# cure-lab/MotionCraft

Measured on AMD Instinct MI355X. Metric: sampled SMPL-X frames/sec (196-frame seq, 1000-step DDPM), higher is better.
Workload: dtype f32

## Files before the change

motioncraft_amd/csrc/mc_ctx.h:

```cpp
#pragma once
#include <map>
#include <mutex>
#include <string>
#include <vector>

#include "../../include/motioncraft_amd.h"
#include "mc_common.h"
#include "mc_gemm.h"
#include "mc_kernels.h"
#include "mc_chain.h"
#include "mc_half.h"
#include "mc_options.h"
#include "mc_params.h"

struct mc_model {
    mc_model_config cfg;
    ParamStore params{""};
    std::map<std::string, HalfW> half;
    std::mutex half_mu;
    size_t half_bytes = 0;
    bool finalized = false;
    int Cp = 0;
};

// ... 40 lines not shown
    const float* mask = nullptr;
    float* mask_own = nullptr;
    int* t_orig;
    float *te, *e1, *emb, *semb, *ss;
    RouteBufs rb;
    int device = 0;
    int coop_reserved = 0;
    bool prof_on = false;
    std::vector<ProfRec> prof;
    bool have_cond = false;
    hipStream_t side = nullptr;
    bool xpad_ready = false;
    hipEvent_t ev_fork = nullptr, ev_join = nullptr;
    hipEvent_t ev_side = nullptr;
    hipEvent_t ev_stag = nullptr;
    bool no_alias = false;
    bool defer_last_gemm = false;
    static constexpr int SIDE_CAND = 4;
    hipStream_t side_cand[SIDE_CAND] = {nullptr, nullptr, nullptr, nullptr};
    hipStream_t side_for = nullptr;
    bool side_picked = false;
    float side_probe_ms[SIDE_CAND] = {0.f, 0.f, 0.f, 0.f};
    static constexpr int SIDE_MEMO = 4;
    hipStream_t side_memo_for[SIDE_MEMO] = {nullptr, nullptr, nullptr, nullptr};
    int side_memo_pick[SIDE_MEMO] = {-1, -1, -1, -1};
    int side_memo_n = 0;
    int* gstep = nullptr;
    SamplerCoefs* gcoefs = nullptr;
    bool graph_mode = false;
    hipGraph_t graph = nullptr;
// ... 37 lines not shown
```

motioncraft_amd/csrc/mc_kernels.h:

```cpp
#pragma once
#include <hip/hip_runtime.h>
#include <stdint.h>
#include "mc_options.h"

struct TwinAlias {
    const int* split_flag = nullptr;
    long from = 0;
};

int mc_launch_ln_rows(const float* X, long ldx, int x_col, const float* gamma, const float* beta,
                      const float* add, int add_mod, float* Y, long ldy, long rows, int L, hipStream_t s);
struct StepRef {
    const int* ptr = nullptr;
    long stride = 0;
};
int mc_launch_film_rows(const float* Y1, const float* Y2, const float* gamma, const float* beta,
                        const float* ss, float* A, long rows, int D, hipStream_t s, TwinAlias y1_alias = TwinAlias(), long row0 = 0,
                        StepRef step = StepRef(), int y1_parts = 1, long y1_pstride = 0,
                        int planes = 0, long plane_stride = 0);
int mc_launch_timestep_embedding(const int* t_orig, float* te, int S, int D, hipStream_t s);
int mc_launch_silu(const float* X, float* Y, long n, hipStream_t s);
int mc_launch_add_rows(float* out, const float* a, const float* b, const float* bias, long rows, int D, hipStream_t s);
int mc_launch_softmax_rows_small(const float* W, float* out, int rows, int cols, hipStream_t s);

// ... 67 lines not shown
    int max_tiles;
    uint32_t tie_xor = 0xFFFFFFFFu;
};
size_t mc_route_state_ints(int E);
bool mc_route_is_small(const McOptions& o, long N);
bool mc_route_cleans_counts(const McOptions& o, long N);
size_t mc_route_barrier_offset();
size_t mc_route_error_offset();
int mc_route_coop_wgs(long N);
int mc_route_coop_slots(int dev);
bool mc_route_coop_reserve(int dev, int nwg);
void mc_route_coop_release(int dev, int nwg);
size_t mc_route_barrier_ints();
int mc_launch_gate_finish(const float* proj, const float* sim_n, const float* logit_scale, long N, int E,
                          RouteBufs rb, hipStream_t s);
int mc_launch_route(long N, long Nsrc, long gsplit, int E, int capacity, RouteBufs rb, const McOptions& o, hipStream_t s);
const int* mc_route_num_tiles_ptr(const RouteBufs& rb, int group = 0);
const int* mc_route_split_flag_ptr(const RouteBufs& rb);

int mc_launch_body(const float* mf, long ldmf, const float* qkv, const float* wsm, float* ys,
                   long frames, int H, int L, int G, hipStream_t s, TwinAlias alias = TwinAlias(), long frame0 = 0);
int mc_launch_temporal(const float* mf, const float* tf, const float* mask, float* yt,
                       int b0, int nb, int B, int T, int Nt, int H, int L, hipStream_t s, const int* twin_flag = nullptr,
                       long lsplit_max = 96,
                       bool pair = false,
                       bool skip_text = false);
```

motioncraft_amd/csrc/mc_model.hip:

```cpp
#include "mc_ctx.h"

namespace {

template <class T>
int ws_alloc(mc_ctx* c, T** p, size_t n) {
    void* d = nullptr;
    size_t bytes = (n * sizeof(T) + 255) & ~(size_t)255;
    if (bytes == 0) bytes = 256;
    MC_HIP(hipMalloc(&d, bytes));
    c->allocs.push_back(d);
    c->bytes += (int64_t)bytes;
    *p = (T*)d;
    return MC_OK;
}

int bind_moe(const mc_model* m, const std::string& pre, int din, int dout, int seq_rows, MoeW* w) {
    const int64_t E = m->cfg.num_experts;
    w->din = din;
    w->dout = dout;
    return m->params.bind({{&w->emb, pre + "emb", (int64_t)seq_rows * din},       {&w->gate_w, pre + "gate_w", 256 * din},
                           {&w->gate_b, pre + "gate_b", 256},                      {&w->sim_n, pre + "sim_n", 256 * E},
                           {&w->sim_nT, pre + "sim_nT", 32 * 256},                 {&w->scale, pre + "scale", 1},
                           {&w->fc1_w, pre + "fc1_w", E * 4 * din * din},          {&w->fc1_b, pre + "fc1_b", E * 4 * din},
                           {&w->fc2_wt, pre + "fc2_wt", E * din * 4 * din},        {&w->fc2_b, pre + "fc2_b", E * din},
// ... 162 lines not shown
    {"temporal_split", "MC_TEMPORAL_SPLIT", nullptr, &McOptions::temporal_split, 96},
    {"big_tokens", "MC_BIG_TOKENS", nullptr, &McOptions::big_tokens, 65536},
    {"rowchain_split", "MC_ROWCHAIN_SPLIT", nullptr, &McOptions::rowchain_split, 20480},
    {"gemm_tune", "MC_GEMM_TUNE", nullptr, &McOptions::gemm_tune, kTuneDefault, check_tune},
    {"small_tile_n", "MC_SMALL_TILE_N", nullptr, &McOptions::small_tile_n, 0,
     [](long v) -> std::string { return v == 0 || v == 48 || v == 64 || v == 96 ? "" : "small_tile_n: 0 (per-launch choice), 48, 64 or 96"; }},
    {"gemm_wp_grid", "MC_GEMM_WP_GRID", nullptr, &McOptions::gemm_wp_grid, 512},
    {"half_min_rows", "MC_HALF_MIN_ROWS", nullptr, &McOptions::half_min_rows, 512},
    {"gate_small", "MC_GATE_SMALL", nullptr, &McOptions::gate_small, 12000},
    {"split_expert", "MC_SPLIT_EXPERT", nullptr, &McOptions::split_expert, 0},
    {"split_sffn", "MC_SPLIT_SFFN", nullptr, &McOptions::split_sffn, 0},
    {"route_reg", "MC_ROUTE_REG", nullptr, &McOptions::route_reg, 1},
    {"route_coop", "MC_ROUTE_COOP", nullptr, &McOptions::route_coop, 1, nullptr, route_coop_hook},
    {"route_small", "MC_ROUTE_SMALL_CTX", "MC_ROUTE_SMALL", &McOptions::route_small, 20480,
     [](long v) -> std::string { return v >= 0 && v <= 131072 ? "" : "route_small: 0 .. 131072 pairs (the one-workgroup kernels hold at most 131072)"; }},
    {"route_per", nullptr, nullptr, &McOptions::route_per, 0,
     [](long v) -> std::string { return v == 0 || v == 10 || v == 16 ? "" : "route_per: 0 (default), 10 or 16"; }},
    {"dbg_delay_us", nullptr, nullptr, &McOptions::dbg_delay_us, 0,
     [](long v) -> std::string { return v >= -100000 && v <= 100000 ? "" : "dbg_delay_us: -100000 .. 100000"; }},
};

int seed_options(McOptions& o) {
    for (const OptionDef& d : kOptions) {
        const char *var = nullptr, *e = nullptr;
        for (const char* v : {d.env, d.env_alt})
            if (v && !e && (e = getenv(v))) var = v;
        const std::string why = e && d.check ? d.check(atol(e)) : "";
        MC_REQUIRE(why.empty(), "%s=%s: %s", var, e, why.c_str());
        o.*d.field = e ? atol(e) : d.dflt;
    }
// ... 59 lines not shown
    probe.m = m;
    int r = bind_weights(&probe);
    if (r != MC_OK) return r;
    m->finalized = true;
    return MC_OK;
}

int mc_ctx_create(mc_model* m, int32_t batch, int32_t frames, int32_t max_steps, mc_ctx** out) {
    MC_REQUIRE(m && out, "null argument");
    MC_REQUIRE(m->finalized, "model not finalized");
    MC_REQUIRE(batch >= 1 && frames >= 1 && frames <= m->cfg.max_seq_len, "bad batch/frames (%d, %d)", batch, frames);
    MC_REQUIRE(max_steps >= 1, "max_steps < 1");
    const mc_model_config& g = m->cfg;
    mc_ctx* c = new mc_ctx();
    if (int r = seed_options(c->opt)) { mc_ctx_destroy(c); return r; }
    c->m = m;
    c->B = batch;
    c->T = frames;
    c->maxS = max_steps;
    const int L = g.latent_dim, H = g.num_parts, D = L * H, F = g.ffn_dim, Te = g.time_embed_dim, Dt = g.text_latent_dim;
    const long B2 = 2L * batch;
    c->rows = B2 * frames;
    c->N = c->rows * H;
    c->Ntxt = B2 * g.max_text_len;
    int r = bind_weights(c);
    if (r == MC_OK) r = build_ctx_weights(c);
    if (r != MC_OK) { mc_ctx_destroy(c); return r; }
    bool cand_ok = true;
    for (int k = 0; k < mc_ctx::SIDE_CAND; ++k) cand_ok = cand_ok && hipStreamCreateWithFlags(&c->side_cand[k], hipStreamNonBlocking) == hipSuccess;
    c->side = c->side_cand[0];
    for (hipEvent_t* e : {&c->ev_fork, &c->ev_join, &c->ev_side, &c->ev_stag}) cand_ok = cand_ok && hipEventCreateWithFlags(e, hipEventDisableTiming) == hipSuccess;
    if (!cand_ok) {
        mc_set_error("could not create the side stream / events");
        mc_ctx_destroy(c);
        return MC_ERR_HIP;
    }
    const long Nmax = c->N > c->Ntxt ? c->N : c->Ntxt;
    const size_t zsz = (size_t)(c->N * L > c->Ntxt * Dt ? c->N * L : c->Ntxt * Dt);
    const size_t hsz = (size_t)(2 * c->N * 4 * L > 2 * c->Ntxt * 4 * Dt ? 2 * c->N * 4 * L : 2 * c->Ntxt * 4 * Dt);
#define WS(p, n) do { if ((r = ws_alloc(c, &(p), (size_t)(n))) != MC_OK) { mc_ctx_destroy(c); return r; } } while (0)
    WS(c->h, c->rows * D);
    WS(c->z, zsz);
    WS(c->proj, Nmax * 256);
    WS(c->hbuf, hsz);
    c->hbuf_cap = hsz;
    if (chain_on(c, kChainMlp) && mc_mlp_supported(L, 4 * L)) c->hbuf_floats = hsz;
// ... 51 lines not shown
    c->graph_multistep = false;
    c->graph_k1.clear();
}
static void prof_clear(mc_ctx* c) {
    for (auto& p : c->prof) { if (p.e0) (void)hipEventDestroy(p.e0); if (p.e1) (void)hipEventDestroy(p.e1); }
    c->prof.clear();
}

void mc_ctx_destroy(mc_ctx* c) {
    if (!c) return;
    graph_release(c);
    if (c->coop_reserved) { mc_route_coop_release(c->device, c->coop_reserved); c->coop_reserved = 0; }
    prof_clear(c);
    for (int k = 0; k < mc_ctx::SIDE_CAND; ++k)
        if (c->side_cand[k]) { (void)hipStreamSynchronize(c->side_cand[k]); (void)hipStreamDestroy(c->side_cand[k]); }
    for (hipEvent_t e : {c->ev_fork, c->ev_join, c->ev_side, c->ev_stag})
        if (e) (void)hipEventDestroy(e);
    for (void* p : c->allocs) (void)hipFree(p);
    delete c;
}

int64_t mc_ctx_workspace_bytes(const mc_ctx* c) { return c ? (int64_t)(c->bytes + (c->prec != MC_PREC_F32 ? c->m->half_bytes : 0)) : 0; }

int mc_ctx_check(mc_ctx* c, void* stream) {
    MC_REQUIRE(c, "null context");
    int flag = 0;
    MC_HIP(hipMemcpyAsync(&flag, c->rb.state + mc_route_error_offset(), sizeof(int), hipMemcpyDeviceToHost, (hipStream_t)stream));
    MC_HIP(hipStreamSynchronize((hipStream_t)stream));
    if (flag != 0) {
        mc_set_error("the cooperative routing kernel's grid barrier timed out (its workgroups were not all resident: another process "
                     "is holding the GPU with barrier kernels of its own); the results of this context are invalid -- destroy it and "
// ... 409 lines not shown
    else if (n == "emb") { p = c->emb; cnt = (int64_t)c->S * g.time_embed_dim; }
    else if (n == "ss") { p = c->ss + (long)layer * c->maxS * 2 * D; cnt = (int64_t)c->S * 2 * D; }
    else if (n == "tf") { p = c->tf + (long)layer * c->Ntxt * 2 * L; cnt = c->Ntxt * 2 * L; }
    else if (n == "idx") { p = c->rb.idx; cnt = 2 * c->N; }
    else if (n == "gate") { p = c->rb.gate; cnt = 2 * c->N; }
    else if (n == "comb_w") { p = c->rb.comb_w; cnt = 2 * c->N; }
    else if (n == "key") { p = c->rb.key; cnt = c->N; }
    else if (n == "hc" && c->hc) { p = c->hc; cnt = c->rows * D; }
    else if (n == "cb" && c->cb) { p = c->cb; cnt = c->rows * D; }
    else if (n == "cap_idx" && c->cap_idx) { p = c->cap_idx + (long)layer * 2 * c->N; cnt = 2 * c->N; }
    else if (n == "cap_w" && c->cap_w) { p = c->cap_w + (long)layer * 2 * c->N; cnt = 2 * c->N; }
    else if (n == "x0_hist") {
        if (!c->x0_hist) { mc_set_error("buffer 'x0_hist' does not exist before the context's first multistep (mode 2) call"); return MC_ERR_STATE; }
        p = c->x0_hist; cnt = (int64_t)c->B * c->T * g.input_feats;
    }
    else if (n == "route_split") { p = const_cast<int*>(mc_route_split_flag_ptr(c->rb)); cnt = 1; }
    else { mc_set_error("unknown buffer '%s'", name); return MC_ERR_ARG; }
    *dev_ptr = p;
    *numel = cnt;
    return MC_OK;
}

int mc_op_gemm(const float* a, const float* w, const float* bias, const float* res, float* cdev, int32_t M, int32_t N,
               int32_t K, int32_t ldw, int32_t act, void* stream) {
    MC_REQUIRE(a && w && cdev && M > 0 && N > 0 && K > 0 && K % 4 == 0 && ldw % 4 == 0 && ldw >= K, "bad gemm args");
    return dense(nullptr, a, K, w, ldw, bias, res, N, cdev, N, M, N, K, act, (hipStream_t)stream);
}

int mc_op_gemm_strided(int32_t mode, int32_t groups, const mc_gemm_strided* a, void* stream) {
    MC_REQUIRE(a && (mode == GM_PLAIN || mode == GM_ENC) && groups >= 1, "gemm_strided: mode %d (0 plain, 4 encoder), groups %d", mode, groups);
// ... 125 lines not shown
```

motioncraft_amd/csrc/mc_options.h:

```cpp
#pragma once

enum ChainBit {
    kChainMlp = 0,
    kChainGate = 1,
    kChainRowchain = 2,
    kChainTwin = 4,
    kChainTwoStreams = 5,
    kChainGroupExperts = 6,
    kChainDeferTail = 7,
    kChainTwinAlias = 8,
    kChainCtrlGroups = 9,
    kChainProjQkv = 10,
    kChainTailGrouped = 11,
    kChainSffnPartials = 12,
    kChainDynSlices = 13,
    kChainSideBody = 14,
    kChainPqBody = 15,
    kChainTwinSplit = 16,
    kChainFilmPlanes = 17,
    kChainMlpDma = 18,
    kChainPadX = 19,
    kChainTemporalHalf = 20,
    kChainTailOnePass = 21,
    kChainTemporalPair = 22,
    kChainSkipText = 24,
    kChainStagger = 26,
    kChainResidualPre = 27,
    kChainFragMajor = 29,
    kChainBits = 30,
};
constexpr long kChainRetired = 1L << 3 | 1L << 23 | 1L << 25 | 1L << 28;
constexpr long kChainDefault = ((1L << kChainBits) - 1) & ~kChainRetired;
static_assert(kChainDefault == 763363319, "the default chain mask is public ABI");

struct McOptions {
    long chain, small_gemm_rows, split_rows_expert, split_rows_sffn, temporal_split, big_tokens, rowchain_split;
    long gemm_tune, small_tile_n, gemm_wp_grid, half_min_rows, gate_small, split_expert, split_sffn;
    long route_reg, route_coop, route_small, route_per, dbg_delay_us;
};

const McOptions* mc_process_options();
```

motioncraft_amd/csrc/mc_route.hip:

```cpp
#include "mc_common.h"
#include "mc_kernels.h"
#include <stdlib.h>

namespace {

constexpr int MAXE = 16;
constexpr int MAXP = 2 * MAXE;
constexpr int TILE_ROWS = 128;

enum {
    ST_CNT = 0,
    ST_KEPT = ST_CNT + MAXP,
    ST_FILL = ST_KEPT + 2 * MAXE,
    ST_OFF = ST_FILL + 2 * MAXE,
    ST_ACTIVE = ST_OFF + 2 * MAXE + 1,
    ST_RANK = ST_ACTIVE + MAXP,
    ST_ANY = ST_RANK + MAXP,
    ST_NTILES = ST_ANY + 1,
    ST_DONE = ST_NTILES + 2,
    ST_SPLIT = ST_DONE + 1,
    ST_PREFIX = ST_DONE + 2,
    ST_HIST = ST_PREFIX + 2 * MAXP,
    ST_BAR = (ST_HIST + MAXP * 256 + 31) / 32 * 32,
    ST_TOTAL = ST_BAR + 17 * 32
};

__device__ __forceinline__ unsigned long long composite(uint32_t key, uint32_t tok, uint32_t tie_xor) {
    return ((unsigned long long)key << 32) | (unsigned long long)(tok ^ tie_xor);
}

__global__ __launch_bounds__(256) void gate_finish_k(const float* __restrict__ proj, const float* __restrict__ sim_n,
                                                     const float* __restrict__ logit_scale, long N, int E,
                                                     int* __restrict__ idx, float* __restrict__ gate,
                                                     uint32_t* __restrict__ key, int* __restrict__ state) {
    __shared__ float s_sim[256 * MAXE];
    __shared__ int s_cnt[MAXP];
    for (int i = threadIdx.x; i < 256 * MAXE; i += 256) {
        const int j = i / MAXE, e = i % MAXE;
// ... 28 lines not shown
        if (e == 0) {
            const float den = fmaxf(m1 + m2, 1.1920928955078125e-07f);
            idx[tok * 2] = c1;
            idx[tok * 2 + 1] = c2;
            gate[tok * 2] = m1 / den;
            gate[tok * 2 + 1] = m2 / den;
            key[tok] = __float_as_uint(m1);
            atomicAdd(&s_cnt[c1], 1);
            atomicAdd(&s_cnt[MAXE + c2], 1);
        }
    }
    __syncthreads();
    if (threadIdx.x < MAXP && s_cnt[threadIdx.x]) atomicAdd(&state[ST_CNT + threadIdx.x], s_cnt[threadIdx.x]);
}

__global__ void route_init_k(int* __restrict__ state, int E, int capacity, int cnt_mul) {
    const int p = threadIdx.x;
    __shared__ int any;
    if (p == 0) any = 0;
    __syncthreads();
    if (p < MAXP) {
        const int choice = p / MAXE, e = p % MAXE;
        int act = 0, rank = 0;
        if (e < E) {
            const int c0 = state[ST_CNT + e] * cnt_mul;
            const int cnt = state[ST_CNT + p] * cnt_mul;
            const int limit = choice == 0 ? capacity : capacity - c0;
            if (limit <= 0) act = cnt > 0 ? -1 : 0;
            else if (cnt > limit) { act = 1; rank = limit; }
        }
        state[ST_ACTIVE + p] = act;
        state[ST_RANK + p] = rank;
        state[ST_PREFIX + 2 * p] = 0;
        state[ST_PREFIX + 2 * p + 1] = 0;
        if (act == 1) atomicOr(&any, 1);
    }
    for (int i = threadIdx.x; i < MAXP * 256; i += blockDim.x) state[ST_HIST + i] = 0;
    if (threadIdx.x < 2 * MAXE) { state[ST_KEPT + threadIdx.x] = 0; state[ST_FILL + threadIdx.x] = 0; }
    if (threadIdx.x < 2) state[ST_DONE + threadIdx.x] = 0;
    __syncthreads();
    if (p == 0) state[ST_ANY] = any;
}

__global__ __launch_bounds__(256) void route_hist_k(const int* __restrict__ idx, const uint32_t* __restrict__ key,
                                                    long N, long Nsrc, int* __restrict__ state, int pass, uint32_t tie_xor) {
    if (state[ST_ANY] == 0) return;
    __shared__ int h[MAXP * 256];
    __shared__ int s_act[MAXP];
    __shared__ unsigned long long s_pre[MAXP];
    for (int i = threadIdx.x; i < MAXP * 256; i += 256) h[i] = 0;
    if (threadIdx.x < MAXP) {
        s_act[threadIdx.x] = state[ST_ACTIVE + threadIdx.x];
        s_pre[threadIdx.x] = ((unsigned long long)(uint32_t)state[ST_PREFIX + 2 * threadIdx.x] << 32) |
                             (uint32_t)state[ST_PREFIX + 2 * threadIdx.x + 1];
    }
    __syncthreads();
// ... 142 lines not shown
            lp[i] = atomicAdd(&s_cnt[le[i]], 1);
        }
    }
    __syncthreads();
    if (threadIdx.x < 2 * MAXE && s_cnt[threadIdx.x])
        s_base[threadIdx.x] = state[ST_OFF + threadIdx.x] + atomicAdd(&state[ST_FILL + threadIdx.x], s_cnt[threadIdx.x]);
    __syncthreads();
#pragma unroll
    for (int i = 0; i < PER; ++i) {
        if (le[i] >= 0) {
            const long a = a0 + i;
            const int slot = s_base[le[i]] + lp[i];
            src_row[slot] = (int)(a >> 1);
            dst_row[slot] = (int)a;
        }
    }
}

__device__ __forceinline__ int ld_state(const int* p) { return __hip_atomic_load(p, __ATOMIC_RELAXED, __HIP_MEMORY_SCOPE_AGENT); }

constexpr int BAR_STRIDE = 32, BAR_INTS = 17 * BAR_STRIDE;
constexpr unsigned BAR_SPIN_LIMIT = 1u << 23;
template <class F>
__device__ __forceinline__ bool grid_sync(int* bar, int nwg, int* s_last, int* s_gen, F&& last_hook) {
    const int grp = (int)(blockIdx.x & 7), ngrp = nwg < 8 ? nwg : 8, members = (nwg - grp + 7) >> 3;
    int* cnt = bar + BAR_STRIDE * (1 + grp);
    int* gen = bar + BAR_STRIDE * (9 + grp);
    __syncthreads();
    if (threadIdx.x == 0) {
        *s_gen = __hip_atomic_load(gen, __ATOMIC_RELAXED, __HIP_MEMORY_SCOPE_AGENT);
// ... 589 lines not shown
    cached[dev].store(v);
    return v;
}
bool mc_route_coop_reserve(int dev, int nwg) {
    if (nwg <= 0 || dev < 0 || dev >= 64) return false;
    const int slots = mc_route_coop_slots(dev);
    int cur = g_coop_reserved[dev].load();
    while (cur + nwg <= slots)
        if (g_coop_reserved[dev].compare_exchange_weak(cur, cur + nwg)) return true;
    return false;
}
void mc_route_coop_release(int dev, int nwg) {
    if (nwg > 0 && dev >= 0 && dev < 64) g_coop_reserved[dev].fetch_sub(nwg);
}
const int* mc_route_num_tiles_ptr(const RouteBufs& rb, int group) { return rb.state + ST_NTILES + group; }
const int* mc_route_split_flag_ptr(const RouteBufs& rb) { return rb.state + ST_SPLIT; }

int mc_launch_gate_finish(const float* proj, const float* sim_n, const float* logit_scale, long N, int E,
                          RouteBufs rb, hipStream_t s) {
    MC_REQUIRE(E >= 2 && E <= MAXE, "gate: num_experts=%d unsupported (2..16)", E);
    MC_HIP(hipMemsetAsync(rb.state, 0, sizeof(int) * (ST_CNT + MAXP), s));
    int blocks = cdiv(N, 16);
    if (blocks > 4096) blocks = 4096;
    hipLaunchKernelGGL(gate_finish_k, dim3(blocks), dim3(256), 0, s, proj, sim_n, logit_scale, N, E, rb.idx, rb.gate,
                       rb.key, rb.state);
    MC_LAUNCH_CHECK();
    return MC_OK;
}

int mc_launch_route(long N, long Nsrc, long gsplit, int E, int capacity, RouteBufs rb, const McOptions& o, hipStream_t s) {
    MC_REQUIRE(Nsrc == N || 2 * Nsrc == N, "route: Nsrc=%ld must be N or N/2 (N=%ld)", Nsrc, N);
    MC_REQUIRE(Nsrc == N || rb.tie_xor == 0xFFFFFFFFu, "route: the twin mode needs the stable tie order (a twin must rank right behind its original)");
    if (mc_route_is_small(o, N)) {
#define MC_ROUTE_SMALL(KERNEL)                                                                                                       \
    hipLaunchKernelGGL(KERNEL, dim3(1), dim3(SMALL_THREADS), 0, s, rb.idx, rb.gate, rb.key, N, Nsrc, gsplit, E, capacity,   \
                       (int)(N / Nsrc), rb.comb_w, rb.state, rb.src_row, rb.dst_row, rb.tile_group, rb.tile_row0, rb.tile_nrows,        \
                       rb.max_tiles, rb.tie_xor)
        if (o.route_reg && 2 * N <= 10L * SMALL_THREADS) MC_ROUTE_SMALL(route_small_k<10>);
        else if (o.route_reg && 2 * N <= 20L * SMALL_THREADS) MC_ROUTE_SMALL(route_small_k<20>);
        else MC_ROUTE_SMALL(route_small_stream_k);
#undef MC_ROUTE_SMALL
        MC_LAUNCH_CHECK();
        return MC_OK;
    }
    if (o.route_coop && 2 * N <= COOP_MAX_WG * 256 * COOP_PER) {
        const int per = o.route_per ? (int)o.route_per : (cdiv(2 * N, 256L * COOP_PER) > 256 ? 16 : 10);
        const int nwg = cdiv(2 * N, 256L * per);
#define MC_ROUTE_COOP(P)                                                                                                             \
    hipLaunchKernelGGL(route_coop_k<P>, dim3(nwg), dim3(256), 0, s, rb.idx, rb.gate, rb.key, N, Nsrc, gsplit, E, capacity, (int)(N / Nsrc), \
                       rb.comb_w, rb.state, rb.src_row, rb.dst_row, rb.tile_group, rb.tile_row0, rb.tile_nrows, rb.max_tiles, rb.tie_xor,  \
                       N <= 65536 ? 1 : 0)
        if (per == 16) MC_ROUTE_COOP(16); else MC_ROUTE_COOP(10);
#undef MC_ROUTE_COOP
        MC_LAUNCH_CHECK();
        return MC_OK;
    }
    hipLaunchKernelGGL(route_init_k, dim3(1), dim3(256), 0, s, rb.state, E, capacity, (int)(N / Nsrc));
    int blocks = cdiv(2 * N, 256 * 8);
    if (blocks > 1024) blocks = 1024;
    if (blocks < 1) blocks = 1;
    for (int pass = 0; pass < 8; ++pass) {
        hipLaunchKernelGGL(route_hist_k, dim3(blocks), dim3(256), 0, s, rb.idx, rb.key, N, Nsrc, rb.state, pass, rb.tie_xor);
    }
    hipLaunchKernelGGL(route_keep_k, dim3(blocks), dim3(256), 0, s, rb.idx, rb.gate, rb.key, N, Nsrc, gsplit, rb.comb_w, rb.state, rb.tie_xor);
    hipLaunchKernelGGL(route_plan_k, dim3(1), dim3(256), 0, s, rb.state, E, rb.tile_group, rb.tile_row0, rb.tile_nrows,
                       rb.max_tiles);
    hipLaunchKernelGGL(route_fill_k, dim3(cdiv(2 * Nsrc, 256 * 8)), dim3(256), 0, s, rb.idx, rb.comb_w, Nsrc, gsplit, rb.state,
                       rb.src_row, rb.dst_row);
    MC_LAUNCH_CHECK();
    return MC_OK;
}
```

motioncraft_amd/csrc/mc_step.hip:

```cpp
#include "mc_ctx.h"

bool use_half(const mc_ctx* c) { return c->prec != MC_PREC_F32 && c->rows > c->opt.half_min_rows; }
static const HalfW* half_planes(const mc_ctx* c, const HalfW* hw) { return hw && hw->hi && use_half(c) ? hw : nullptr; }
static bool split3(const mc_ctx* c) { return c->prec == MC_PREC_F16X3; }

static bool twin_aliased(const mc_ctx* c, bool twin) { return twin && chain_on(c, kChainTwinAlias) && !c->no_alias; }
static TwinAlias twin_alias(const mc_ctx* c, bool twin, bool tokens) {
    return twin_aliased(c, twin) ? TwinAlias{mc_route_split_flag_ptr(c->rb), (tokens ? c->N : c->rows) / 2} : TwinAlias();
}

template <class Args>
static void set_tile_map(const mc_ctx* c, int group, Args& a) {
    const long to = (long)group * c->rb.max_tiles;
    a.tile_group = c->rb.tile_group + to; a.tile_row0 = c->rb.tile_row0 + to; a.tile_nrows = c->rb.tile_nrows + to;
    a.num_tiles = mc_route_num_tiles_ptr(c->rb, group);
}

static int dbg_hold(const mc_ctx* c, hipStream_t pos, hipStream_t neg) {
    const long us = c->opt.dbg_delay_us;
    return us == 0 ? MC_OK : mc_launch_spin((us > 0 ? us : -us) * 100, us > 0 ? pos : neg);
}

int dense(const mc_ctx* c, const float* A, long lda, const float* W, long ldw, const float* bias, const float* R, long ldr,
          float* C, long ldc, long M, int N, int K, int act, hipStream_t s) {
// ... 91 lines not shown
    p.Y = Y; p.ldy = ldy; p.tok0 = tok0; p.N = tok0 + ntok; p.L = w.din; p.Nout = w.dout;
    p.twin_from = twin_from;
    p.alias = alias;
    return p;
}
static int moe_proj(const mc_ctx* c, const MoeW& w, float* Y, long ldy, long tok0, long ntok, long twin_from, const TwinAlias& alias, hipStream_t s) {
    if (proj_chained(c, w)) return mc_launch_rowchain(0, proj_chain_args(c, w, Y, ldy, tok0, ntok, twin_from, alias), s);
    GemmArgs p;
    mc_gemm_opts(c->opt, p);
    p.A = c->y2 + 2 * tok0 * w.din; p.lda = w.din; p.comb_w = c->rb.comb_w + 2 * tok0;
    p.W = w.proj_w; p.ldw = w.din; p.bias = w.proj_b;
    p.C = Y + tok0 * ldy; p.ldc = ldy; p.M = (int)ntok; p.N = w.dout; p.K = w.din;
    return mc_launch_gemm(GM_COMB, p, 1, 0, s);
}

int run_moe(mc_ctx* c, const MoeW& w, const float* z, long Ntok, float* out, long ldout, bool gated, bool twin, long gsplit,
            hipStream_t s, const HalfW* hw, const HalfW* hw2) {
    const mc_model_config& g = c->m->cfg;
    const int E = g.num_experts, din = w.din;
    int r;
    if (!gated) {
        if ((r = dense(c, z, din, w.gate_w, din, w.gate_b, nullptr, 0, c->proj, 256, Ntok, 256, din, ACT_NONE, s))) return r;
        if ((r = mc_launch_gate_finish(c->proj, w.sim_n, w.scale, Ntok, E, c->rb, s))) return r;
    }
    const int capacity = g.topk * (int)((double)g.capacity_factor * (double)((Ntok + E - 1) / E));
    c->cnt_clean = false;
    c->led_nsrc = twin ? Ntok / 2 : Ntok;
    c->led_gsplit = gsplit;
    if ((r = mc_launch_route(Ntok, twin ? Ntok / 2 : Ntok, gsplit, E, capacity, c->rb, c->opt, s))) return r;
    c->cnt_clean = mc_route_cleans_counts(c->opt, Ntok);
    if (gsplit < Ntok) return MC_OK;
    if ((r = moe_experts(c, w, z, Ntok, 0, s, hw, hw2))) return r;
    if (!out) return MC_OK;
    return moe_proj(c, w, out, ldout, 0, Ntok, twin ? Ntok / 2 : 0, TwinAlias(), s);
}

bool a_holds_planes(const mc_ctx* c) {
    const long D = (long)c->m->cfg.latent_dim * c->m->cfg.num_parts;
    return use_half(c) && chain_on(c, kChainFilmPlanes) && D % 128 == 0 && c->rows * D * 2 < (1L << 31);
}

// ... 242 lines not shown
    MC_HIP(hipStreamWaitEvent(s, c->ev_side, 0));
    return MC_OK;
}

static int run_layer(mc_ctx* c, int i, float* hs, int step, bool twin_ok, int split, hipStream_t s) {
    const mc_model_config& g = c->m->cfg;
    const int L = g.latent_dim, H = g.num_parts;
    const LayerW& w = c->lw[i];
    int r;
    const bool fused_gate = chain_on(c, kChainGate) && mc_mlp_supported(L, 32);
    const bool twin = twin_ok && fused_gate && chain_on(c, kChainRowchain) && chain_on(c, kChainTwin) && (c->N % 2 == 0) &&
                      c->rb.tie_xor == 0xFFFFFFFFu;
    const long half = (long)c->B * c->T;
    const long sub_rows = ((long)c->B / 2) * c->T;
    const bool twin_split = twin && split == 2 && chain_on(c, kChainGroupExperts) && chain_on(c, kChainTwinAlias) && chain_on(c, kChainTwinSplit) && !c->no_alias && sub_rows > 0;
    if (fused_gate) {
        GateArgs ga;
        ga.X = hs; ga.ldx = L; ga.gamma = w.norm_g; ga.beta = w.norm_b; ga.emb = w.mm.emb; ga.emb_mod = c->T * H;
        ga.Z = c->z; ga.Wp = w.mm.gate_w; ga.bp = w.mm.gate_b; ga.sim_nT = w.mm.sim_nT; ga.logit_scale = w.mm.scale;
        ga.E = g.num_experts; ga.L = L; ga.small_tokens = c->opt.gate_small;
        ga.idx = c->rb.idx; ga.gate = c->rb.gate; ga.key = c->rb.key; ga.cnt = c->rb.state;
        if (split == 2 && (!twin || twin_split)) {
            if (!c->cnt_clean) MC_HIP(hipMemsetAsync(ga.cnt, 0, sizeof(int) * 32, s));
            c->cnt_clean = false;
            if ((r = side_fork(c, s))) return r;
            ga.zero_cnt = 0;
            const long cut = twin_split ? sub_rows * H : half * H;
            ga.tok0 = 0; ga.N = cut;
            if ((r = mc_launch_gate(ga, s))) return r;
            ga.tok0 = cut; ga.N = twin_split ? half * H : c->N;
            if ((r = mc_launch_gate(ga, c->side))) return r;
        } else {
            ga.N = twin ? c->N / 2 : c->N;
            ga.zero_cnt = c->cnt_clean ? 0 : 1;
            c->cnt_clean = false;
            if ((r = mc_launch_gate(ga, s))) return r;
        }
        if (split == 2 && (r = side_join(c, s))) return r;
    } else {
        if ((r = mc_launch_ln_rows(hs, L, 0, w.norm_g, w.norm_b, w.mm.emb, c->T * H, c->z, L, c->N, L, s))) return r;
    }
    const bool grouped = split == 2 && chain_on(c, kChainGroupExperts);
    const long gsplit = twin_split ? sub_rows * H : grouped ? half * H : c->N;
    if ((r = run_moe(c, w.mm, c->z, c->N, nullptr, 0, fused_gate, twin, gsplit, s, &w.h_fc1, &w.h_fc2))) return r;
    if (c->cap_idx) {
        if (twin) {
            MC_HIP(hipMemcpyAsync(c->cap_idx + (long)i * 2 * c->N, c->rb.idx, sizeof(int) * c->N, hipMemcpyDeviceToDevice, s));
            MC_HIP(hipMemcpyAsync(c->cap_idx + (long)i * 2 * c->N + c->N, c->rb.idx, sizeof(int) * c->N, hipMemcpyDeviceToDevice, s));
        } else {
            MC_HIP(hipMemcpyAsync(c->cap_idx + (long)i * 2 * c->N, c->rb.idx, sizeof(int) * 2 * c->N, hipMemcpyDeviceToDevice, s));
        }
        MC_HIP(hipMemcpyAsync(c->cap_w + (long)i * 2 * c->N, c->rb.comb_w, sizeof(float) * 2 * c->N, hipMemcpyDeviceToDevice, s));
    }
    const bool evstag = split == 2 && chain_on(c, kChainStagger) && !use_half(c) && L == 128;
    if (split) {
        if (twin_split) {
            if ((r = side_fork(c, s))) return r;
            if ((r = moe_experts(c, w.mm, c->z, c->N, 0, s, &w.h_fc1, &w.h_fc2))) return r;
            if ((r = moe_experts(c, w.mm, c->z, c->N, 1, c->side, &w.h_fc1, &w.h_fc2))) return r;
            auto front = [&](long row0, long nrows, hipStream_t sk) {
                const int e = layer_proj(c, i, twin, row0, nrows, sk);
                return e ? e : layer_body(c, i, twin, row0, nrows, sk);
            };
            if ((r = front(0, sub_rows, s))) return r;
            if ((r = front(sub_rows, half - sub_rows, c->side))) return r;
            MC_HIP(hipEventRecord(c->ev_join, s));
            MC_HIP(hipEventRecord(c->ev_side, c->side));
            MC_HIP(hipStreamWaitEvent(c->side, c->ev_join, 0));
            MC_HIP(hipStreamWaitEvent(s, c->ev_side, 0));
            if ((r = front(half, half, c->side))) return r;
            if ((r = layer_temporal(c, i, twin, 0, half, s))) return r;
            if ((r = layer_temporal(c, i, twin, half, half, c->side))) return r;
        } else {
            if (grouped && twin) {
                if ((r = moe_experts(c, w.mm, c->z, c->N, 0, s, &w.h_fc1, &w.h_fc2))) return r;
                if ((r = side_fork(c, s))) return r;
            } else {
                if ((r = side_fork(c, s))) return r;
                if (grouped) {
                    if ((r = moe_experts(c, w.mm, c->z, c->N, 0, s, &w.h_fc1, &w.h_fc2))) return r;
                    if ((r = moe_experts(c, w.mm, c->z, c->N, 1, c->side, &w.h_fc1, &w.h_fc2))) return r;
                }
            }
            if ((r = layer_rows(c, i, twin, 0, half, s, s))) return r;
            if (twin_aliased(c, twin)) {
                MC_HIP(hipEventRecord(c->ev_join, s));
                MC_HIP(hipStreamWaitEvent(c->side, c->ev_join, 0));
            }
            if ((r = layer_rows(c, i, twin, half, half, c->side, c->side))) return r;
        }
        if ((r = dbg_hold(c, c->side, s))) return r;
        if ((r = layer_rows_tail(c, i, hs, step, twin, 0, half, s, evstag ? c->ev_stag : nullptr, nullptr))) return r;
        if ((r = layer_rows_tail(c, i, hs, step, twin, half, half, c->side, nullptr, evstag ? c->ev_stag : nullptr))) return r;
        return split == 1 ? side_join(c, s) : MC_OK;
    }
    const bool side_temporal = c->side && c->N <= c->opt.big_tokens;
    if ((r = layer_rows(c, i, twin, 0, 2 * half, s, side_temporal ? c->side : s))) return r;
    return layer_rows_tail(c, i, hs, step, twin, 0, 2 * half, s);
}

int denoise_impl(mc_ctx* c, const float* x_t, int32_t step, float* out2_dev, int32_t stop_after, void* stream, const SeedArgs* seed) {
    MC_REQUIRE(c && x_t, "null argument");
    MC_REQUIRE(c->have_cond, "mc_ctx_set_condition not called");
    MC_REQUIRE(step >= 0 && step < c->S, "step_index %d outside the %d-step schedule", step, c->S);
// ... 134 lines not shown
```

Baseline: 659.1.

## Start MoE experts per group before global route selection completes

Adds an early-routing path. Each token group runs its own gate and fills its own per-group route plan (new fill-group kernel and separate count slots), then starts its expert GEMMs on its own stream. The global capacity selection runs afterwards in a select-only mode. The aim is to overlap gating, routing and expert compute across the main and side streams instead of serialising on a full route before any expert starts. It adds new events and cross-stream waits, and it disables the path by default for latent_dim 64. Experts now run on the pre-capacity plan, so correctness depends on how the later selection reconciles with it.

```diff
diff --git a/motioncraft_amd/csrc/mc_ctx.h b/motioncraft_amd/csrc/mc_ctx.h
--- a/motioncraft_amd/csrc/mc_ctx.h
+++ b/motioncraft_amd/csrc/mc_ctx.h
@@ -78,6 +78,8 @@
     hipEvent_t ev_fork = nullptr, ev_join = nullptr;
     hipEvent_t ev_side = nullptr;
     hipEvent_t ev_stag = nullptr;
+    hipEvent_t ev_gate1 = nullptr, ev_sel = nullptr, ev_front = nullptr;
+    bool early_clean = false;
     bool no_alias = false;
     bool defer_last_gemm = false;
     static constexpr int SIDE_CAND = 4;
diff --git a/motioncraft_amd/csrc/mc_kernels.h b/motioncraft_amd/csrc/mc_kernels.h
--- a/motioncraft_amd/csrc/mc_kernels.h
+++ b/motioncraft_amd/csrc/mc_kernels.h
@@ -105,7 +105,10 @@
 size_t mc_route_barrier_ints();
 int mc_launch_gate_finish(const float* proj, const float* sim_n, const float* logit_scale, long N, int E,
                           RouteBufs rb, hipStream_t s);
-int mc_launch_route(long N, long Nsrc, long gsplit, int E, int capacity, RouteBufs rb, const McOptions& o, hipStream_t s);
+int mc_launch_route(long N, long Nsrc, long gsplit, int E, int capacity, RouteBufs rb, const McOptions& o, hipStream_t s, bool select_only = false);
+int* mc_route_group_counts(const RouteBufs& rb, int group);
+int mc_launch_route_fill_group(int group, long tok0, long ntok, int E, RouteBufs rb, hipStream_t s);
+int mc_route_early_reset(const RouteBufs& rb, hipStream_t s);
 const int* mc_route_num_tiles_ptr(const RouteBufs& rb, int group = 0);
 const int* mc_route_split_flag_ptr(const RouteBufs& rb);
 
diff --git a/motioncraft_amd/csrc/mc_model.hip b/motioncraft_amd/csrc/mc_model.hip
--- a/motioncraft_amd/csrc/mc_model.hip
+++ b/motioncraft_amd/csrc/mc_model.hip
@@ -200,6 +200,8 @@
     {"route_coop", "MC_ROUTE_COOP", nullptr, &McOptions::route_coop, 1, nullptr, route_coop_hook},
     {"route_small", "MC_ROUTE_SMALL_CTX", "MC_ROUTE_SMALL", &McOptions::route_small, 20480,
      [](long v) -> std::string { return v >= 0 && v <= 131072 ? "" : "route_small: 0 .. 131072 pairs (the one-workgroup kernels hold at most 131072)"; }},
+    {"route_early", "MC_ROUTE_EARLY", nullptr, &McOptions::route_early, 1,
+     [](long v) -> std::string { return v == 0 || v == 1 ? "" : "route_early: 0 or 1"; }},
     {"route_per", nullptr, nullptr, &McOptions::route_per, 0,
      [](long v) -> std::string { return v == 0 || v == 10 || v == 16 ? "" : "route_per: 0 (default), 10 or 16"; }},
     {"dbg_delay_us", nullptr, nullptr, &McOptions::dbg_delay_us, 0,
@@ -289,6 +291,7 @@
     const mc_model_config& g = m->cfg;
     mc_ctx* c = new mc_ctx();
     if (int r = seed_options(c->opt)) { mc_ctx_destroy(c); return r; }
+    if (m->cfg.latent_dim == 64 && !getenv("MC_ROUTE_EARLY")) c->opt.route_early = 0;
     c->m = m;
     c->B = batch;
     c->T = frames;
@@ -304,7 +307,7 @@
     bool cand_ok = true;
     for (int k = 0; k < mc_ctx::SIDE_CAND; ++k) cand_ok = cand_ok && hipStreamCreateWithFlags(&c->side_cand[k], hipStreamNonBlocking) == hipSuccess;
     c->side = c->side_cand[0];
-    for (hipEvent_t* e : {&c->ev_fork, &c->ev_join, &c->ev_side, &c->ev_stag}) cand_ok = cand_ok && hipEventCreateWithFlags(e, hipEventDisableTiming) == hipSuccess;
+    for (hipEvent_t* e : {&c->ev_fork, &c->ev_join, &c->ev_side, &c->ev_stag, &c->ev_gate1, &c->ev_sel, &c->ev_front}) cand_ok = cand_ok && hipEventCreateWithFlags(e, hipEventDisableTiming) == hipSuccess;
     if (!cand_ok) {
         mc_set_error("could not create the side stream / events");
         mc_ctx_destroy(c);
@@ -386,7 +389,7 @@
     prof_clear(c);
     for (int k = 0; k < mc_ctx::SIDE_CAND; ++k)
         if (c->side_cand[k]) { (void)hipStreamSynchronize(c->side_cand[k]); (void)hipStreamDestroy(c->side_cand[k]); }
-    for (hipEvent_t e : {c->ev_fork, c->ev_join, c->ev_side, c->ev_stag})
+    for (hipEvent_t e : {c->ev_fork, c->ev_join, c->ev_side, c->ev_stag, c->ev_gate1, c->ev_sel, c->ev_front})
         if (e) (void)hipEventDestroy(e);
     for (void* p : c->allocs) (void)hipFree(p);
     delete c;
@@ -826,6 +829,12 @@
         if (!c->x0_hist) { mc_set_error("buffer 'x0_hist' does not exist before the context's first multistep (mode 2) call"); return MC_ERR_STATE; }
         p = c->x0_hist; cnt = (int64_t)c->B * c->T * g.input_feats;
     }
+    else if (n == "src_row") { p = c->rb.src_row; cnt = 2 * c->N; }
+    else if (n == "dst_row") { p = c->rb.dst_row; cnt = 2 * c->N; }
+    else if (n == "tile_group") { p = c->rb.tile_group; cnt = 2L * c->rb.max_tiles; }
+    else if (n == "tile_row0") { p = c->rb.tile_row0; cnt = 2L * c->rb.max_tiles; }
+    else if (n == "tile_nrows") { p = c->rb.tile_nrows; cnt = 2L * c->rb.max_tiles; }
+    else if (n == "num_tiles") { p = const_cast<int*>(mc_route_num_tiles_ptr(c->rb, 0)); cnt = 2; }
     else if (n == "route_split") { p = const_cast<int*>(mc_route_split_flag_ptr(c->rb)); cnt = 1; }
     else { mc_set_error("unknown buffer '%s'", name); return MC_ERR_ARG; }
     *dev_ptr = p;
diff --git a/motioncraft_amd/csrc/mc_options.h b/motioncraft_amd/csrc/mc_options.h
--- a/motioncraft_amd/csrc/mc_options.h
+++ b/motioncraft_amd/csrc/mc_options.h
@@ -36,7 +36,7 @@
 struct McOptions {
     long chain, small_gemm_rows, split_rows_expert, split_rows_sffn, temporal_split, big_tokens, rowchain_split;
     long gemm_tune, small_tile_n, gemm_wp_grid, half_min_rows, gate_small, split_expert, split_sffn;
-    long route_reg, route_coop, route_small, route_per, dbg_delay_us;
+    long route_reg, route_coop, route_small, route_early, route_per, dbg_delay_us;
 };
 
 const McOptions* mc_process_options();
diff --git a/motioncraft_amd/csrc/mc_route.hip b/motioncraft_amd/csrc/mc_route.hip
--- a/motioncraft_amd/csrc/mc_route.hip
+++ b/motioncraft_amd/csrc/mc_route.hip
@@ -21,7 +21,8 @@
     ST_SPLIT = ST_DONE + 1,
     ST_PREFIX = ST_DONE + 2,
     ST_HIST = ST_PREFIX + 2 * MAXP,
-    ST_BAR = (ST_HIST + MAXP * 256 + 31) / 32 * 32,
+    ST_CNT1 = ST_HIST + MAXP * 256,
+    ST_BAR = (ST_CNT1 + MAXP + 31) / 32 * 32,
     ST_TOTAL = ST_BAR + 17 * 32
 };
 
@@ -80,7 +81,7 @@
     if (threadIdx.x < MAXP && s_cnt[threadIdx.x]) atomicAdd(&state[ST_CNT + threadIdx.x], s_cnt[threadIdx.x]);
 }
 
-__global__ void route_init_k(int* __restrict__ state, int E, int capacity, int cnt_mul) {
+__global__ void route_init_k(int* __restrict__ state, int E, int capacity, int cnt_mul, int early) {
     const int p = threadIdx.x;
     __shared__ int any;
     if (p == 0) any = 0;
@@ -89,8 +90,8 @@
         const int choice = p / MAXE, e = p % MAXE;
         int act = 0, rank = 0;
         if (e < E) {
-            const int c0 = state[ST_CNT + e] * cnt_mul;
-            const int cnt = state[ST_CNT + p] * cnt_mul;
+            const int c0 = (state[ST_CNT + e] + (early ? state[ST_CNT1 + e] : 0)) * cnt_mul;
+            const int cnt = (state[ST_CNT + p] + (early ? state[ST_CNT1 + p] : 0)) * cnt_mul;
             const int limit = choice == 0 ? capacity : capacity - c0;
             if (limit <= 0) act = cnt > 0 ? -1 : 0;
             else if (cnt > limit) { act = 1; rank = limit; }
@@ -106,6 +107,7 @@
     if (threadIdx.x < 2) state[ST_DONE + threadIdx.x] = 0;
     __syncthreads();
     if (p == 0) state[ST_ANY] = any;
+    if (early && p < MAXP) { state[ST_CNT + p] = 0; state[ST_CNT1 + p] = 0; }
 }
 
 __global__ __launch_bounds__(256) void route_hist_k(const int* __restrict__ idx, const uint32_t* __restrict__ key,
@@ -278,6 +280,64 @@
             src_row[slot] = (int)(a >> 1);
             dst_row[slot] = (int)a;
         }
+    }
+}
+
+__global__ __launch_bounds__(256) void route_fill_group_k(const int* __restrict__ idx, const int* __restrict__ cnt, long tok0, long ntok, int E,
+                                                          int* __restrict__ cursor, int* __restrict__ num_tiles, int* __restrict__ tile_group,
+                                                          int* __restrict__ tile_row0, int* __restrict__ tile_nrows, int max_tiles,
+                                                          int* __restrict__ src_row, int* __restrict__ dst_row) {
+    constexpr int PER = 8;
+    __shared__ int s_off[MAXE + 1], s_t0[MAXE + 1], s_cnt[MAXE], s_base[MAXE];
+    const long a_begin = 2 * tok0, a_end = 2 * (tok0 + ntok);
+    if (threadIdx.x < MAXE) s_cnt[threadIdx.x] = 0;
+    if (threadIdx.x == 0) {
+        long off = a_begin;
+        int nt = 0;
+        for (int e = 0; e < MAXE; ++e) {
+            s_off[e] = (int)off;
+            s_t0[e] = nt;
+            const int c = e < E ? cnt[e] + cnt[MAXE + e] : 0;
+            off += c;
+            nt += (c + TILE_ROWS - 1) / TILE_ROWS;
+        }
+        s_off[MAXE] = (int)off;
+        s_t0[MAXE] = nt;
+        if (blockIdx.x == 0) *num_tiles = min(nt, max_tiles);
+    }
+    __syncthreads();
+    if (blockIdx.x == 0)
+        for (int e = 0; e < E; ++e) {
+            const int t1 = min(s_t0[e + 1], max_tiles);
+            for (int t = s_t0[e] + threadIdx.x; t < t1; t += blockDim.x) {
+                const int r = (t - s_t0[e]) * TILE_ROWS;
+                tile_group[t] = e;
+                tile_row0[t] = s_off[e] + r;
+                tile_nrows[t] = min(TILE_ROWS, s_off[e + 1] - s_off[e] - r);
+            }
+        }
+    const long a0 = a_begin + ((long)blockIdx.x * 256 + threadIdx.x) * PER;
+    int le[PER], lp[PER];
+#pragma unroll
+    for (int i = 0; i < PER; ++i) {
+        const long a = a0 + i;
+        le[i] = -1;
+        if (a < a_end) {
+            const int e = idx[a];
+            if (e >= 0 && e < E) { le[i] = e; lp[i] = atomicAdd(&s_cnt[e], 1); }
+        }
+    }
+    __syncthreads();
+    if (threadIdx.x < MAXE && s_cnt[threadIdx.x]) s_base[threadIdx.x] = s_off[threadIdx.x] + atomicAdd(&cursor[threadIdx.x], s_cnt[threadIdx.x]);
+    __syncthreads();
+#pragma unroll
+    for (int i = 0; i < PER; ++i) {
+        if (le[i] < 0) continue;
+        const long a = a0 + i;
+        const long slot = (long)s_base[le[i]] + lp[i];
+        if (slot < a_begin || slot >= a_end) continue;
+        src_row[slot] = (int)(a >> 1);
+        dst_row[slot] = (int)a;
     }
 }
 
@@ -897,6 +957,25 @@
     if (nwg > 0 && dev >= 0 && dev < 64) g_coop_reserved[dev].fetch_sub(nwg);
 }
 const int* mc_route_num_tiles_ptr(const RouteBufs& rb, int group) { return rb.state + ST_NTILES + group; }
+int* mc_route_group_counts(const RouteBufs& rb, int group) { return rb.state + (group ? ST_CNT1 : ST_CNT); }
+
+int mc_route_early_reset(const RouteBufs& rb, hipStream_t s) {
+    MC_HIP(hipMemsetAsync(rb.state, 0, sizeof(int) * ST_OFF, s));
+    MC_HIP(hipMemsetAsync(rb.state + ST_CNT1, 0, sizeof(int) * MAXP, s));
+    return MC_OK;
+}
+
+int mc_launch_route_fill_group(int group, long tok0, long ntok, int E, RouteBufs rb, hipStream_t s) {
+    MC_REQUIRE(group == 0 || group == 1, "route fill: group %d", group);
+    MC_REQUIRE(E >= 2 && E <= MAXE && tok0 >= 0 && ntok >= 0 && 2 * (tok0 + ntok) < (1L << 31), "route fill: bad range (%ld, %ld)", tok0, ntok);
+    const long to = (long)group * rb.max_tiles;
+    const int blocks = ntok > 0 ? (int)cdiv(2 * ntok, 256L * 8) : 1;
+    hipLaunchKernelGGL(route_fill_group_k, dim3(blocks), dim3(256), 0, s, rb.idx, mc_route_group_counts(rb, group), tok0, ntok, E,
+                       rb.state + ST_FILL + group * MAXE, rb.state + ST_NTILES + group, rb.tile_group + to, rb.tile_row0 + to,
+                       rb.tile_nrows + to, rb.max_tiles, rb.src_row, rb.dst_row);
+    MC_LAUNCH_CHECK();
+    return MC_OK;
+}
 const int* mc_route_split_flag_ptr(const RouteBufs& rb) { return rb.state + ST_SPLIT; }
 
 int mc_launch_gate_finish(const float* proj, const float* sim_n, const float* logit_scale, long N, int E,
@@ -911,9 +990,10 @@
     return MC_OK;
 }
 
-int mc_launch_route(long N, long Nsrc, long gsplit, int E, int capacity, RouteBufs rb, const McOptions& o, hipStream_t s) {
+int mc_launch_route(long N, long Nsrc, long gsplit, int E, int capacity, RouteBufs rb, const McOptions& o, hipStream_t s, bool select_only) {
     MC_REQUIRE(Nsrc == N || 2 * Nsrc == N, "route: Nsrc=%ld must be N or N/2 (N=%ld)", Nsrc, N);
     MC_REQUIRE(Nsrc == N || rb.tie_xor == 0xFFFFFFFFu, "route: the twin mode needs the stable tie order (a twin must rank right behind its original)");
+    MC_REQUIRE(!select_only || !mc_route_is_small(o, N), "route: the selection-only mode is not for the one-workgroup sizes");
     if (mc_route_is_small(o, N)) {
 #define MC_ROUTE_SMALL(KERNEL)                                                                                                       \
     hipLaunchKernelGGL(KERNEL, dim3(1), dim3(SMALL_THREADS), 0, s, rb.idx, rb.gate, rb.key, N, Nsrc, gsplit, E, capacity,   \
@@ -926,7 +1006,7 @@
         MC_LAUNCH_CHECK();
         return MC_OK;
     }
-    if (o.route_coop && 2 * N <= COOP_MAX_WG * 256 * COOP_PER) {
+    if (!select_only && o.route_coop && 2 * N <= COOP_MAX_WG * 256 * COOP_PER) {
         const int per = o.route_per ? (int)o.route_per : (cdiv(2 * N, 256L * COOP_PER) > 256 ? 16 : 10);
         const int nwg = cdiv(2 * N, 256L * per);
 #define MC_ROUTE_COOP(P)                                                                                                             \
@@ -938,7 +1018,7 @@
         MC_LAUNCH_CHECK();
         return MC_OK;
     }
-    hipLaunchKernelGGL(route_init_k, dim3(1), dim3(256), 0, s, rb.state, E, capacity, (int)(N / Nsrc));
+    hipLaunchKernelGGL(route_init_k, dim3(1), dim3(256), 0, s, rb.state, E, capacity, (int)(N / Nsrc), select_only ? 1 : 0);
     int blocks = cdiv(2 * N, 256 * 8);
     if (blocks > 1024) blocks = 1024;
     if (blocks < 1) blocks = 1;
@@ -946,6 +1026,7 @@
         hipLaunchKernelGGL(route_hist_k, dim3(blocks), dim3(256), 0, s, rb.idx, rb.key, N, Nsrc, rb.state, pass, rb.tie_xor);
     }
     hipLaunchKernelGGL(route_keep_k, dim3(blocks), dim3(256), 0, s, rb.idx, rb.gate, rb.key, N, Nsrc, gsplit, rb.comb_w, rb.state, rb.tie_xor);
+    if (select_only) { MC_LAUNCH_CHECK(); return MC_OK; }
     hipLaunchKernelGGL(route_plan_k, dim3(1), dim3(256), 0, s, rb.state, E, rb.tile_group, rb.tile_row0, rb.tile_nrows,
                        rb.max_tiles);
     hipLaunchKernelGGL(route_fill_k, dim3(cdiv(2 * Nsrc, 256 * 8)), dim3(256), 0, s, rb.idx, rb.comb_w, Nsrc, gsplit, rb.state,
diff --git a/motioncraft_amd/csrc/mc_step.hip b/motioncraft_amd/csrc/mc_step.hip
--- a/motioncraft_amd/csrc/mc_step.hip
+++ b/motioncraft_amd/csrc/mc_step.hip
@@ -129,6 +129,11 @@
     return mc_launch_gemm(GM_COMB, p, 1, 0, s);
 }
 
+static int moe_capacity(const mc_model_config& g, long Ntok) {
+    const int E = g.num_experts;
+    return g.topk * (int)((double)g.capacity_factor * (double)((Ntok + E - 1) / E));
+}
+
 int run_moe(mc_ctx* c, const MoeW& w, const float* z, long Ntok, float* out, long ldout, bool gated, bool twin, long gsplit,
             hipStream_t s, const HalfW* hw, const HalfW* hw2) {
     const mc_model_config& g = c->m->cfg;
@@ -138,8 +143,9 @@
         if ((r = dense(c, z, din, w.gate_w, din, w.gate_b, nullptr, 0, c->proj, 256, Ntok, 256, din, ACT_NONE, s))) return r;
         if ((r = mc_launch_gate_finish(c->proj, w.sim_n, w.scale, Ntok, E, c->rb, s))) return r;
     }
-    const int capacity = g.topk * (int)((double)g.capacity_factor * (double)((Ntok + E - 1) / E));
+    const int capacity = moe_capacity(g, Ntok);
     c->cnt_clean = false;
+    c->early_clean = false;
     c->led_nsrc = twin ? Ntok / 2 : Ntok;
     c->led_gsplit = gsplit;
     if ((r = mc_launch_route(Ntok, twin ? Ntok / 2 : Ntok, gsplit, E, capacity, c->rb, c->opt, s))) return r;
@@ -412,13 +418,42 @@
     const long half = (long)c->B * c->T;
     const long sub_rows = ((long)c->B / 2) * c->T;
     const bool twin_split = twin && split == 2 && chain_on(c, kChainGroupExperts) && chain_on(c, kChainTwinAlias) && chain_on(c, kChainTwinSplit) && !c->no_alias && sub_rows > 0;
+    const bool grouped = split == 2 && chain_on(c, kChainGroupExperts);
+    const long gsplit = twin_split ? sub_rows * H : grouped ? half * H : c->N;
+    const bool early = fused_gate && grouped && c->opt.route_early != 0 && !mc_route_is_small(c->opt, c->N);
     if (fused_gate) {
         GateArgs ga;
         ga.X = hs; ga.ldx = L; ga.gamma = w.norm_g; ga.beta = w.norm_b; ga.emb = w.mm.emb; ga.emb_mod = c->T * H;
         ga.Z = c->z; ga.Wp = w.mm.gate_w; ga.bp = w.mm.gate_b; ga.sim_nT = w.mm.sim_nT; ga.logit_scale = w.mm.scale;
         ga.E = g.num_experts; ga.L = L; ga.small_tokens = c->opt.gate_small;
         ga.idx = c->rb.idx; ga.gate = c->rb.gate; ga.key = c->rb.key; ga.cnt = c->rb.state;
-        if (split == 2 && (!twin || twin_split)) {
+        if (early) {
+            const bool two = !twin || twin_split;
+            const long nsrc = twin ? c->N / 2 : c->N;
+            const int E = g.num_experts;
+            if (!(c->cnt_clean && c->early_clean) && (r = mc_route_early_reset(c->rb, s))) return r;
+            c->cnt_clean = c->early_clean = false;
+            c->led_nsrc = nsrc;
+            c->led_gsplit = gsplit;
+            if (two && (r = side_fork(c, s))) return r;
+            ga.zero_cnt = 0;
+            ga.tok0 = 0; ga.N = gsplit; ga.cnt = mc_route_group_counts(c->rb, 0);
+            if ((r = mc_launch_gate(ga, s))) return r;
+            if ((r = mc_launch_route_fill_group(0, 0, gsplit, E, c->rb, s))) return r;
+            if ((r = moe_experts(c, w.mm, c->z, c->N, 0, s, &w.h_fc1, &w.h_fc2))) return r;
+            if (two) {
+                ga.tok0 = gsplit; ga.N = nsrc; ga.cnt = mc_route_group_counts(c->rb, 1);
+                if ((r = mc_launch_gate(ga, c->side))) return r;
+                if ((r = mc_launch_route_fill_group(1, gsplit, nsrc - gsplit, E, c->rb, c->side))) return r;
+                MC_HIP(hipEventRecord(c->ev_gate1, c->side));
+                if ((r = moe_experts(c, w.mm, c->z, c->N, 1, c->side, &w.h_fc1, &w.h_fc2))) return r;
+                MC_HIP(hipStreamWaitEvent(s, c->ev_gate1, 0));
+            } else if ((r = mc_launch_route_fill_group(1, gsplit, 0, E, c->rb, s))) return r;
+            if ((r = mc_launch_route(c->N, nsrc, gsplit, E, moe_capacity(g, c->N), c->rb, c->opt, s, true))) return r;
+            c->cnt_clean = c->early_clean = true;
+            MC_HIP(hipEventRecord(c->ev_sel, s));
+            if (two) MC_HIP(hipStreamWaitEvent(c->side, c->ev_sel, 0));
+        } else if (split == 2 && (!twin || twin_split)) {
             if (!c->cnt_clean) MC_HIP(hipMemsetAsync(ga.cnt, 0, sizeof(int) * 32, s));
             c->cnt_clean = false;
             if ((r = side_fork(c, s))) return r;
@@ -434,13 +469,11 @@
             c->cnt_clean = false;
             if ((r = mc_launch_gate(ga, s))) return r;
         }
-        if (split == 2 && (r = side_join(c, s))) return r;
+        if (split == 2 && !early && (r = side_join(c, s))) return r;
     } else {
         if ((r = mc_launch_ln_rows(hs, L, 0, w.norm_g, w.norm_b, w.mm.emb, c->T * H, c->z, L, c->N, L, s))) return r;
     }
-    const bool grouped = split == 2 && chain_on(c, kChainGroupExperts);
-    const long gsplit = twin_split ? sub_rows * H : grouped ? half * H : c->N;
-    if ((r = run_moe(c, w.mm, c->z, c->N, nullptr, 0, fused_gate, twin, gsplit, s, &w.h_fc1, &w.h_fc2))) return r;
+    if (!early && (r = run_moe(c, w.mm, c->z, c->N, nullptr, 0, fused_gate, twin, gsplit, s, &w.h_fc1, &w.h_fc2))) return r;
     if (c->cap_idx) {
         if (twin) {
             MC_HIP(hipMemcpyAsync(c->cap_idx + (long)i * 2 * c->N, c->rb.idx, sizeof(int) * c->N, hipMemcpyDeviceToDevice, s));
@@ -453,9 +486,11 @@
     const bool evstag = split == 2 && chain_on(c, kChainStagger) && !use_half(c) && L == 128;
     if (split) {
         if (twin_split) {
-            if ((r = side_fork(c, s))) return r;
-            if ((r = moe_experts(c, w.mm, c->z, c->N, 0, s, &w.h_fc1, &w.h_fc2))) return r;
-            if ((r = moe_experts(c, w.mm, c->z, c->N, 1, c->side, &w.h_fc1, &w.h_fc2))) return r;
+            if (!early) {
+                if ((r = side_fork(c, s))) return r;
+                if ((r = moe_experts(c, w.mm, c->z, c->N, 0, s, &w.h_fc1, &w.h_fc2))) return r;
+                if ((r = moe_experts(c, w.mm, c->z, c->N, 1, c->side, &w.h_fc1, &w.h_fc2))) return r;
+            }
             auto front = [&](long row0, long nrows, hipStream_t sk) {
                 const int e = layer_proj(c, i, twin, row0, nrows, sk);
                 return e ? e : layer_body(c, i, twin, row0, nrows, sk);
@@ -467,13 +502,15 @@
             MC_HIP(hipStreamWaitEvent(c->side, c->ev_join, 0));
             MC_HIP(hipStreamWaitEvent(s, c->ev_side, 0));
             if ((r = front(half, half, c->side))) return r;
+            if (early) MC_HIP(hipEventRecord(c->ev_front, c->side));
             if ((r = layer_temporal(c, i, twin, 0, half, s))) return r;
+            if (early) MC_HIP(hipStreamWaitEvent(s, c->ev_front, 0));
             if ((r = layer_temporal(c, i, twin, half, half, c->side))) return r;
         } else {
             if (grouped && twin) {
-                if ((r = moe_experts(c, w.mm, c->z, c->N, 0, s, &w.h_fc1, &w.h_fc2))) return r;
+                if (!early && (r = moe_experts(c, w.mm, c->z, c->N, 0, s, &w.h_fc1, &w.h_fc2))) return r;
                 if ((r = side_fork(c, s))) return r;
-            } else {
+            } else if (!early) {
                 if ((r = side_fork(c, s))) return r;
                 if (grouped) {
                     if ((r = moe_experts(c, w.mm, c->z, c->N, 0, s, &w.h_fc1, &w.h_fc2))) return r;
@@ -486,6 +523,10 @@
                 MC_HIP(hipStreamWaitEvent(c->side, c->ev_join, 0));
             }
             if ((r = layer_rows(c, i, twin, half, half, c->side, c->side))) return r;
+            if (early && twin) {
+                MC_HIP(hipEventRecord(c->ev_front, c->side));
+                MC_HIP(hipStreamWaitEvent(s, c->ev_front, 0));
+            }
         }
         if ((r = dbg_hold(c, c->side, s))) return r;
         if ((r = layer_rows_tail(c, i, hs, step, twin, 0, half, s, evstag ? c->ev_stag : nullptr, nullptr))) return r;
```

After: 666.5, median of 6. 1.01x the previous value.
